# HanielUlises/GCN-GrabCut

Measured on AMD Instinct MI355X. Metric: images/sec end-to-end mask (DUTS-shape batch), higher is better.
Workload: dtype f32

## Files before the change

### gcn-grabcut_amd/csrc/ggc_gc.h

```cpp
#pragma once
#include "ggc_internal.h"

namespace ggc {

constexpr int DINF = 1 << 29;

struct GcDims { int B, H, W, P, n_chunks; };

__device__ __forceinline__ int dir_dx(int dir) { return (dir == 0 || dir == 4 || dir == 7) ? -1 : ((dir == 1 || dir == 5 || dir == 6) ? 1 : 0); }
__device__ __forceinline__ int dir_dy(int dir) { return (dir == 2 || dir == 4 || dir == 6) ? -1 : ((dir == 3 || dir == 5 || dir == 7) ? 1 : 0); }
__device__ __forceinline__ int dir_nb(const GcDims& d, int y, int x, int dir) {
    const int yy = y + dir_dy(dir), xx = x + dir_dx(dir);
    if (xx < 0 || xx >= d.W || yy < 0 || yy >= d.H) return -1;
    return yy * d.W + xx;
}

__host__ __device__ __forceinline__ size_t rc_idx(int dir, size_t i) { return i * 8 + (size_t)dir; }

__device__ __forceinline__ void mf_cold_pixel(size_t i, int32_t tw, const int32_t (&cap)[8], int32_t* __restrict__ rc,
                                              int32_t* __restrict__ ex, int32_t* __restrict__ snk, uint8_t* __restrict__ rmask) {
    int arcs = 0;
    int4* r = reinterpret_cast<int4*>(rc + rc_idx(0, i));
    r[0] = make_int4(cap[0], cap[1], cap[2], cap[3]);
    r[1] = make_int4(cap[4], cap[5], cap[6], cap[7]);
// ... 6 lines not shown

__device__ __forceinline__ void mf_plane_caps(const GcDims& d, int b, int p, const int32_t* __restrict__ nw, int32_t (&cap)[8]) {
    const size_t BP = (size_t)d.B * d.P;
    const int y = p / d.W, x = p % d.W;
    const int32_t* nwb = nw + (size_t)b * d.P;
    const int dirs[4] = {0, 4, 2, 6};
#pragma unroll
    for (int k = 0; k < 4; ++k) {
        const int dir = dirs[k];
        cap[dir] = dir_nb(d, y, x, dir) >= 0 ? nwb[(size_t)k * BP + p] : 0;
        const int q = dir_nb(d, y, x, dir ^ 1);
        cap[dir ^ 1] = q >= 0 ? nwb[(size_t)k * BP + q] : 0;
    }
}

__device__ __forceinline__ void mf_warm_pixel(size_t i, int32_t tw, int32_t tw_old, int32_t* __restrict__ ex,
                                              int32_t* __restrict__ snk) {
    const int32_t bal = (ex[i] - snk[i]) + (tw - tw_old);
    ex[i] = bal > 0 ? bal : 0;
    snk[i] = bal < 0 ? -bal : 0;
}

struct MfControl {
    int32_t* active;
    int32_t* cnt;
    int32_t* lists;
    int32_t* err;
};

int maxflow(ggc_ctx* ctx, hipStream_t st, const GcDims& d, const int32_t* state, int32_t* rc, int32_t* ex,
            int32_t* snk, int32_t* dist, uint8_t* rmask, const MfControl& ctl, bool masks_exact, int& n_open);

constexpr int MF_RT = 32;
constexpr int MF_PT_W = 32, MF_PT_H = 8;
struct MfTiles { int rt_x, rt_y, pt_x, pt_y; };
// ... 13 lines not shown
```

### gcn-grabcut_amd/csrc/ggc_grabcut.hip

```cpp
#include "ggc_gc.h"
#include "ggc_math.h"
#include <algorithm>
#include <cmath>
#include <cstdlib>
#include <vector>

namespace ggc {

constexpr int NCOMP = 5;
constexpr double CAP_SCALE = 262144.0;
constexpr double GAMMA = 50.0, LAMBDA = 9.0 * GAMMA;
constexpr int CHUNK = 1024;


struct Gmm {
    double coef[NCOMP], mean[NCOMP][3], cov[NCOMP][9];
    double inv[NCOMP][3][3], det[NCOMP];
    double isd[NCOMP];
};

__host__ __device__ inline void gmm_prepare(Gmm& g, int ci, double fix) {
    if (!(g.coef[ci] > 0.0)) return;
    double* c = g.cov[ci];
    double d = c[0] * (c[4] * c[8] - c[5] * c[7]) - c[1] * (c[3] * c[8] - c[5] * c[6]) + c[2] * (c[3] * c[7] - c[4] * c[6]);
// ... 3 lines not shown
    }
    g.det[ci] = d;
    g.isd[ci] = 1.0 / sqrt(d);
    const double id = 1.0 / d;
    g.inv[ci][0][0] = (c[4] * c[8] - c[5] * c[7]) * id;
    g.inv[ci][1][0] = -(c[3] * c[8] - c[5] * c[6]) * id;
    g.inv[ci][2][0] = (c[3] * c[7] - c[4] * c[6]) * id;
    g.inv[ci][0][1] = -(c[1] * c[8] - c[2] * c[7]) * id;
    g.inv[ci][1][1] = (c[0] * c[8] - c[2] * c[6]) * id;
    g.inv[ci][2][1] = -(c[0] * c[7] - c[1] * c[6]) * id;
    g.inv[ci][0][2] = (c[1] * c[5] - c[2] * c[4]) * id;
    g.inv[ci][1][2] = -(c[0] * c[5] - c[2] * c[3]) * id;
    g.inv[ci][2][2] = (c[0] * c[4] - c[1] * c[3]) * id;
}

__device__ __forceinline__ double gmm_comp(const Gmm& g, int ci, const uint8_t* px) {
    if (!(g.coef[ci] > 0.0)) return 0.0;
    const double d0 = (double)px[0] - g.mean[ci][0], d1 = (double)px[1] - g.mean[ci][1], d2 = (double)px[2] - g.mean[ci][2];
    const double mult = d0 * (d0 * g.inv[ci][0][0] + d1 * g.inv[ci][1][0] + d2 * g.inv[ci][2][0])
                      + d1 * (d0 * g.inv[ci][0][1] + d1 * g.inv[ci][1][1] + d2 * g.inv[ci][2][1])
                      + d2 * (d0 * g.inv[ci][0][2] + d1 * g.inv[ci][1][2] + d2 * g.inv[ci][2][2]);
    return g.isd[ci] * det_exp(-0.5 * mult);
}
__device__ __forceinline__ double gmm_total(const Gmm& g, const uint8_t* px) {
    double r = 0.0;
    for (int ci = 0; ci < NCOMP; ++ci) r += g.coef[ci] * gmm_comp(g, ci, px);
    return r;
}
__device__ __forceinline__ int gmm_which(const Gmm& g, const uint8_t* px) {
    int k = 0; double mx = 0.0;
    for (int ci = 0; ci < NCOMP; ++ci) { const double p = gmm_comp(g, ci, px); if (p > mx) { k = ci; mx = p; } }
    return k;
}

__device__ __forceinline__ bool is_bg(uint8_t m) { return m == GGC_BGD || m == GGC_PR_BGD; }

__global__ void __launch_bounds__(256) k_gc_flags(GcDims d, const uint8_t* __restrict__ mask, int32_t* __restrict__ flags) {
    const int b = blockIdx.y;
    int f = 0;
    for (int p = blockIdx.x * blockDim.x + threadIdx.x; p < d.P; p += gridDim.x * blockDim.x) {
        const uint8_t m = mask[(size_t)b * d.P + p];
        f |= (m == GGC_FGD) ? 1 : 0;
        f |= (m == GGC_BGD) ? 2 : 0;
        f |= (m > 3) ? 4 : 0;
        f |= is_bg(m) ? 8 : 16;
    }
    for (int o = 32; o > 0; o >>= 1) f |= __shfl_xor(f, o, 64);
    __shared__ int s_f[4];
    if ((threadIdx.x & 63) == 0) s_f[threadIdx.x >> 6] = f;
    __syncthreads();
    if (threadIdx.x == 0) {
        f = s_f[0] | s_f[1] | s_f[2] | s_f[3];
        if (f & ~__hip_atomic_load(&flags[b], __ATOMIC_RELAXED, __HIP_MEMORY_SCOPE_AGENT)) atomicOr(&flags[b], f);
    }
}

__global__ void __launch_bounds__(256) k_gc_promote(GcDims d, const int32_t* __restrict__ flags, uint8_t* __restrict__ mask) {
    const size_t i = (size_t)blockIdx.x * blockDim.x + threadIdx.x;
    if (i >= (size_t)d.B * d.P) return;
    const int f = flags[i / d.P];
    uint8_t m = mask[i];
    if (!(f & 1) && m == GGC_PR_FGD) m = GGC_FGD;
    if (!(f & 2) && m == GGC_PR_BGD) m = GGC_BGD;
    mask[i] = m;
}

__global__ void __launch_bounds__(256) k_gc_rect(GcDims d, const int32_t* __restrict__ rects, uint8_t* __restrict__ mask) {
    const size_t i = (size_t)blockIdx.x * blockDim.x + threadIdx.x;
    if (i >= (size_t)d.B * d.P) return;
    const int b = (int)(i / d.P), p = (int)(i % d.P);
    const int y = p / d.W, x = p % d.W;
    int x0 = rects[4 * b], y0 = rects[4 * b + 1], w = rects[4 * b + 2], h = rects[4 * b + 3];
    if (x0 < 0) { w += x0; x0 = 0; }
    if (y0 < 0) { h += y0; y0 = 0; }
    if (x0 + w > d.W) w = d.W - x0;
    if (y0 + h > d.H) h = d.H - y0;
    mask[i] = (x >= x0 && x < x0 + w && y >= y0 && y < y0 + h) ? GGC_PR_FGD : GGC_BGD;
}

__global__ void k_gc_state(int B, int mode, const int32_t* __restrict__ f1, const int32_t* __restrict__ f2,
                           int32_t* __restrict__ state, int32_t* __restrict__ err) {
    const int b = blockIdx.x * blockDim.x + threadIdx.x;
    if (b >= B) return;
    int s = 0;
    if ((f1[b] | f2[b]) & 4) { *err = 1; s = 1; }
    if (mode == 0 && (f2[b] & 3) != 3) s = 1;
    if (mode != 2 && (f2[b] & 24) != 24) s = 1;
    state[b] = s;
}

__device__ __forceinline__ uint64_t splitmix(uint64_t& s) {
    uint64_t z = (s += 0x9E3779B97F4A7C15ULL);
    z = (z ^ (z >> 30)) * 0xBF58476D1CE4E5B9ULL;
    z = (z ^ (z >> 27)) * 0x94D049BB133111EBULL;
    return z ^ (z >> 31);
}

struct KmState {
    uint64_t rng;
    int64_t n;
    int32_t K;
    int32_t cen_px[NCOMP];
    double cen[NCOMP][3];
};

__global__ void __launch_bounds__(256) k_km_chunks(GcDims d, int k, const uint8_t* __restrict__ img,
                                                   const uint8_t* __restrict__ mask, const int32_t* __restrict__ state,
                                                   const KmState* __restrict__ km, int32_t* __restrict__ d2,
                                                   int64_t* __restrict__ chunk_cnt, int64_t* __restrict__ chunk_d2) {
    __shared__ long long s_cnt[2][4], s_d2[2][4];
    const int b = blockIdx.y, ch = blockIdx.x, tid = threadIdx.x;
    if (state[b]) return;
    const uint8_t* im = img + (size_t)b * d.P * 3;
    long long cnt[2] = {0, 0}, sd[2] = {0, 0};
    for (int t = 0; t < CHUNK / 256; ++t) {
        const int p = ch * CHUNK + t * 256 + tid;
        if (p >= d.P) continue;
        const int c = is_bg(mask[(size_t)b * d.P + p]) ? 0 : 1;
        int v = 0;
        if (k > 0) {
            const KmState& s = km[b * 2 + c];
            if (k - 1 < s.K) {
                const int q = s.cen_px[k - 1];
                int dd = 0;
                for (int ch3 = 0; ch3 < 3; ++ch3) { const int t3 = (int)im[3 * p + ch3] - (int)im[3 * q + ch3]; dd += t3 * t3; }
                v = (k == 1) ? dd : min(d2[(size_t)b * d.P + p], dd);
                d2[(size_t)b * d.P + p] = v;
            } else v = d2[(size_t)b * d.P + p];
        }
        cnt[c] += 1; sd[c] += v;
    }
    for (int c = 0; c < 2; ++c)
        for (int o = 32; o > 0; o >>= 1) { cnt[c] += __shfl_xor(cnt[c], o, 64); sd[c] += __shfl_xor(sd[c], o, 64); }
    if ((tid & 63) == 0) for (int c = 0; c < 2; ++c) { s_cnt[c][tid >> 6] = cnt[c]; s_d2[c][tid >> 6] = sd[c]; }
    __syncthreads();
    if (tid < 2) {
        const size_t o = ((size_t)b * 2 + tid) * d.n_chunks + ch;
        chunk_cnt[o] = s_cnt[tid][0] + s_cnt[tid][1] + s_cnt[tid][2] + s_cnt[tid][3];
        chunk_d2[o] = s_d2[tid][0] + s_d2[tid][1] + s_d2[tid][2] + s_d2[tid][3];
    }
}

__device__ __forceinline__ long long wave_sum64(long long v) {
    for (int o = 32; o > 0; o >>= 1) v += __shfl_xor(v, o, 64);
    return v;
// ... 74 lines not shown
        s.rng = rng;
        s.cen_px[k] = pick;
        for (int ch3 = 0; ch3 < 3; ++ch3) s.cen[k][ch3] = (double)img[((size_t)b * d.P + pick) * 3 + ch3];
    }
}

constexpr int ACC_W = 13;

constexpr int BIN_COPIES = 16, BIN_PX = 4;

__global__ void __launch_bounds__(256) k_km_assign(GcDims d, const uint8_t* __restrict__ img,
                                                   const uint8_t* __restrict__ mask, const int32_t* __restrict__ state,
                                                   const KmState* __restrict__ km, uint8_t* __restrict__ comp,
                                                   unsigned long long* __restrict__ acc, int store_comp) {
    __shared__ unsigned int s_acc[2 * NCOMP * 4 * BIN_COPIES];
    const int b = blockIdx.y, tid = threadIdx.x, cp = tid % BIN_COPIES;
    if (state[b]) return;
    for (int i = tid; i < 2 * NCOMP * 4 * BIN_COPIES; i += 256) s_acc[i] = 0;
    __syncthreads();
#pragma unroll
    for (int j = 0; j < BIN_PX; ++j) {
        const int p = (blockIdx.x * BIN_PX + j) * 256 + tid;
        if (p < d.P) {
            const size_t gp = (size_t)b * d.P + p;
            const int c = is_bg(mask[gp]) ? 0 : 1;
            const uint8_t* px = img + gp * 3;
            int best = 0; double bd = 0.0;
#pragma unroll
            for (int cc = 0; cc < 2; ++cc) {
                if (c != cc) continue;
                const KmState& s = km[b * 2 + cc];
                for (int k = 0; k < s.K; ++k) {
                    const double a0 = (double)px[0] - s.cen[k][0], a1 = (double)px[1] - s.cen[k][1], a2 = (double)px[2] - s.cen[k][2];
                    const double dist = (a0 * a0 + a1 * a1) + a2 * a2;
                    if (k == 0 || dist < bd) { best = k; bd = dist; }
                }
            }
            if (store_comp) comp[gp] = (uint8_t)best;
            unsigned int* a = s_acc + (c * NCOMP + best) * 4 * BIN_COPIES + cp;
            atomicAdd(&a[0], 1u); atomicAdd(&a[BIN_COPIES], (unsigned int)px[0]);
            atomicAdd(&a[2 * BIN_COPIES], (unsigned int)px[1]); atomicAdd(&a[3 * BIN_COPIES], (unsigned int)px[2]);
        }
    }
    __syncthreads();
    for (int i = tid; i < 2 * NCOMP * 4; i += 256) {
        unsigned int v = 0;
#pragma unroll
        for (int k = 0; k < BIN_COPIES; ++k) v += s_acc[i * BIN_COPIES + k];
        if (v) atomicAdd(&acc[((size_t)b * 2 * NCOMP + i / 4) * ACC_W + (i % 4)], (unsigned long long)v);
    }
}

__global__ void k_km_update(int B, const int32_t* __restrict__ state, KmState* __restrict__ km,
                            unsigned long long* __restrict__ acc, int update) {
    const int i = blockIdx.x * blockDim.x + threadIdx.x;
    if (i >= B * 2 * NCOMP) return;
    const int b = i / (2 * NCOMP), c = (i / NCOMP) % 2, k = i % NCOMP;
    unsigned long long* a = acc + (size_t)i * ACC_W;
    if (!state[b] && update && a[0] > 0)
        for (int ch = 0; ch < 3; ++ch) km[b * 2 + c].cen[k][ch] = (double)(long long)a[1 + ch] / (double)(long long)a[0];
    for (int j = 0; j < ACC_W; ++j) a[j] = 0;
}

template <int MODE>
__global__ void __launch_bounds__(256) k_gmm_accum(GcDims d, const uint8_t* __restrict__ img,
                                                   uint8_t* __restrict__ mask, const int32_t* __restrict__ state,
                                                   const Gmm* __restrict__ gmm, const uint8_t* __restrict__ comp,
                                                   const int32_t* __restrict__ dist, unsigned long long* __restrict__ acc) {
    constexpr int LW = 10;
    __shared__ unsigned int s_acc[2 * NCOMP * LW * BIN_COPIES];
    const int b = blockIdx.y, tid = threadIdx.x, cp = tid % BIN_COPIES;
    if (state[b]) return;
    for (int i = tid; i < 2 * NCOMP * LW * BIN_COPIES; i += 256) s_acc[i] = 0;
    __syncthreads();
#pragma unroll
    for (int j = 0; j < BIN_PX; ++j) {
        const int p = (blockIdx.x * BIN_PX + j) * 256 + tid;
        if (p < d.P) {
            const size_t gp = (size_t)b * d.P + p;
            uint8_t m = mask[gp];
            if (MODE == 1 && dist && (m == GGC_PR_BGD || m == GGC_PR_FGD)) {
                const uint8_t m1 = dist[gp] >= DINF ? GGC_PR_FGD : GGC_PR_BGD;
                if (m1 != m) mask[gp] = m = m1;
            }
            const int c = is_bg(m) ? 0 : 1;
            const uint8_t* px = img + gp * 3;
            int ci = 0;
            if (MODE == 1) {
#pragma unroll
                for (int cc = 0; cc < 2; ++cc) if (c == cc) ci = gmm_which(gmm[b * 2 + cc], px);
            } else ci = comp[gp];
            unsigned int* a = s_acc + (c * NCOMP + ci) * LW * BIN_COPIES + cp;
            const unsigned int v0 = px[0], v1 = px[1], v2 = px[2];
            atomicAdd(&a[0], 1u);
            atomicAdd(&a[1 * BIN_COPIES], v0); atomicAdd(&a[2 * BIN_COPIES], v1); atomicAdd(&a[3 * BIN_COPIES], v2);
            atomicAdd(&a[4 * BIN_COPIES], v0 * v0); atomicAdd(&a[5 * BIN_COPIES], v0 * v1); atomicAdd(&a[6 * BIN_COPIES], v0 * v2);
            atomicAdd(&a[7 * BIN_COPIES], v1 * v1); atomicAdd(&a[8 * BIN_COPIES], v1 * v2); atomicAdd(&a[9 * BIN_COPIES], v2 * v2);
        }
    }
    __syncthreads();
    for (int i = tid; i < 2 * NCOMP * ACC_W; i += 256) {
        const int bin = i / ACC_W, slot = i % ACC_W;
        int ls = slot;
        if (slot >= 4) {
            const int r = (slot - 4) / 3, cc = (slot - 4) % 3;
            const int lo = r < cc ? r : cc, hi = r < cc ? cc : r;
            ls = 4 + (lo == 0 ? hi : (lo == 1 ? 2 + hi : 5));
        }
        unsigned int v = 0;
#pragma unroll
        for (int k = 0; k < BIN_COPIES; ++k) v += s_acc[(bin * LW + ls) * BIN_COPIES + k];
        if (v) atomicAdd(&acc[(size_t)b * 2 * NCOMP * ACC_W + i], (unsigned long long)v);
    }
}

__global__ void k_gmm_learn(int B, const int32_t* __restrict__ state, unsigned long long* __restrict__ acc,
                            Gmm* __restrict__ gmm) {
    const int i = blockIdx.x * blockDim.x + threadIdx.x;
    if (i >= B * 2) return;
    unsigned long long* a = acc + (size_t)i * NCOMP * ACC_W;
    if (!state[i / 2]) {
        Gmm& g = gmm[i];
        long long total = 0;
        for (int ci = 0; ci < NCOMP; ++ci) total += (long long)a[ci * ACC_W];
        for (int ci = 0; ci < NCOMP; ++ci) {
            const long long n = (long long)a[ci * ACC_W];
            if (n == 0) { g.coef[ci] = 0.0; continue; }
            const double inv_n = 1.0 / (double)n;
            g.coef[ci] = (double)n / (double)total;
            for (int r = 0; r < 3; ++r) g.mean[ci][r] = (double)(long long)a[ci * ACC_W + 1 + r] * inv_n;
            for (int r = 0; r < 3; ++r)
                for (int c = 0; c < 3; ++c)
                    g.cov[ci][3 * r + c] = (double)(long long)a[ci * ACC_W + 4 + 3 * r + c] * inv_n - g.mean[ci][r] * g.mean[ci][c];
            gmm_prepare(g, ci, 0.01);
        }
    }
    for (int j = 0; j < NCOMP * ACC_W; ++j) a[j] = 0;
}

__global__ void k_gmm_from_model(int B, const double* __restrict__ bgd, const double* __restrict__ fgd, Gmm* __restrict__ gmm) {
    const int i = blockIdx.x * blockDim.x + threadIdx.x;
    if (i >= B * 2) return;
// ... 4 lines not shown
    for (int k = 0; k < 45; ++k) g.cov[k / 9][k % 9] = m[4 * NCOMP + k];
    for (int ci = 0; ci < NCOMP; ++ci) gmm_prepare(g, ci, 0.0);
}

__global__ void k_gmm_to_model(int B, const int32_t* __restrict__ state, const Gmm* __restrict__ gmm,
                               double* __restrict__ bgd, double* __restrict__ fgd) {
    const int i = blockIdx.x * blockDim.x + threadIdx.x;
    if (i >= B * 2 || state[i / 2]) return;
    double* m = (i & 1 ? fgd : bgd) + (size_t)(i / 2) * 65;
    const Gmm& g = gmm[i];
    for (int k = 0; k < NCOMP; ++k) m[k] = g.coef[k];
    for (int k = 0; k < 15; ++k) m[NCOMP + k] = g.mean[k / 3][k % 3];
    for (int k = 0; k < 45; ++k) m[4 * NCOMP + k] = g.cov[k / 9][k % 9];
}

__device__ __forceinline__ bool plane_nb(const GcDims& d, int y, int x, int k, int& q) {
    const int dy = (k == 0) ? 0 : -1, dx = (k == 0 || k == 1) ? -1 : (k == 2 ? 0 : 1);
    const int yy = y + dy, xx = x + dx;
    if (xx < 0 || xx >= d.W || yy < 0) return false;
    q = yy * d.W + xx;
    return true;
}
__device__ __forceinline__ int colour_d2(const uint8_t* a, const uint8_t* b) {
    const int t0 = (int)a[0] - (int)b[0], t1 = (int)a[1] - (int)b[1], t2 = (int)a[2] - (int)b[2];
    return t0 * t0 + t1 * t1 + t2 * t2;
}

__global__ void __launch_bounds__(256) k_beta(GcDims d, const uint8_t* __restrict__ img, unsigned long long* __restrict__ bsum) {
    const int b = blockIdx.y;
    const uint8_t* im = img + (size_t)b * d.P * 3;
    unsigned long long s = 0;
    for (int p = blockIdx.x * blockDim.x + threadIdx.x; p < d.P; p += gridDim.x * blockDim.x) {
        const int y = p / d.W, x = p % d.W;
        for (int k = 0; k < 4; ++k) { int q; if (plane_nb(d, y, x, k, q)) s += (unsigned long long)colour_d2(im + 3 * p, im + 3 * q); }
    }
    for (int o = 32; o > 0; o >>= 1) s += __shfl_xor(s, o, 64);
    if ((threadIdx.x & 63) == 0 && s) atomicAdd(&bsum[b], s);
}

__device__ __forceinline__ double gc_beta(const GcDims& d, unsigned long long bsum) {
    const long long bs = (long long)bsum;
    return bs > 0 ? 1.0 / (2.0 * (double)bs / (double)(4ll * d.W * d.H - 3ll * d.W - 3ll * d.H + 2)) : 0.0;
}
__device__ __forceinline__ int32_t nlink_cap(double beta, bool diagonal, const uint8_t* a, const uint8_t* b) {
    const double gdiv = GAMMA / sqrt(2.0);
    const double wt = (diagonal ? gdiv : GAMMA) * det_exp(-beta * (double)colour_d2(a, b));
    return (int32_t)rint(wt * CAP_SCALE);
}

__global__ void __launch_bounds__(256) k_build_graph(GcDims d, const uint8_t* __restrict__ img,
                                                     const uint8_t* __restrict__ mask, const int32_t* __restrict__ state,
                                                     const Gmm* __restrict__ gmm, const unsigned long long* __restrict__ bsum,
                                                     int32_t* __restrict__ rc, int32_t* __restrict__ ex,
                                                     int32_t* __restrict__ snk, uint8_t* __restrict__ rmask,
                                                     int32_t* __restrict__ tws, int warm) {
    const int b = blockIdx.y, p = blockIdx.x * blockDim.x + threadIdx.x;
    if (p >= d.P || state[b]) return;
    const size_t i = (size_t)b * d.P + p;
    const uint8_t m = mask[i];
    if (warm && (m == GGC_BGD || m == GGC_FGD)) return;
    double dv;
    if (m == GGC_BGD) dv = -LAMBDA;
    else if (m == GGC_FGD) dv = LAMBDA;
    else {
        const uint8_t* px = img + i * 3;
        const double from_src = -det_log(gmm_total(gmm[b * 2 + 0], px));
        const double to_snk = -det_log(gmm_total(gmm[b * 2 + 1], px));
        dv = from_src - to_snk;
        if (dv != dv) dv = 0.0;
        if (dv > LAMBDA) dv = LAMBDA;
        if (dv < -LAMBDA) dv = -LAMBDA;
    }
    const int32_t tw = (int32_t)rint(dv * CAP_SCALE);
    if (warm) mf_warm_pixel(i, tw, tws[i], ex, snk);
    else {
        const uint8_t* im = img + (size_t)b * d.P * 3;
        const double beta = gc_beta(d, bsum[b]);
        const int y = p / d.W, x = p % d.W;
        int32_t cap[8];
#pragma unroll
        for (int dir = 0; dir < 8; ++dir) {
            const int q = dir_nb(d, y, x, dir);
            cap[dir] = q >= 0 ? nlink_cap(beta, dir >= 4, im + 3 * p, im + 3 * q) : 0;
        }
        mf_cold_pixel(i, tw, cap, rc, ex, snk, rmask);
    }
    tws[i] = tw;
}

// ... 17 lines not shown
extern "C" int ggc_grabcut(ggc_ctx* ctx, ggc_stream stream, int B, int H, int W, const uint8_t* image,
                           uint8_t* mask, const int32_t* rects, double* bgd_model, double* fgd_model,
                           int n_iter, int mode, uint64_t seed, uint8_t* binary) {
    if (!ctx) return GGC_E_INVALID_ARG;
    GGC_REQUIRE(ctx, B >= 1 && H >= 1 && W >= 1 && B <= 65535, GGC_E_SHAPE, "bad shape B=%d H=%d W=%d", B, H, W);
    GGC_REQUIRE(ctx, (size_t)H * W < (1u << 28), GGC_E_SHAPE, "image too large");
    GGC_REQUIRE(ctx, image && mask, GGC_E_INVALID_ARG, "null pointer");
    GGC_REQUIRE(ctx, mode >= 0 && mode <= 2, GGC_E_INVALID_ARG, "mode must be 0 (mask), 1 (rect) or 2 (eval)");
    GGC_REQUIRE(ctx, mode != 1 || rects, GGC_E_INVALID_ARG, "mode 1 needs rects");
    GGC_REQUIRE(ctx, mode != 2 || (bgd_model && fgd_model), GGC_E_INVALID_ARG, "mode 2 needs both models");
    GGC_HIP(ctx, hipSetDevice(ctx->device));
    hipStream_t st = reinterpret_cast<hipStream_t>(stream);
    GcDims d{B, H, W, H * W, cdiv((size_t)H * W, CHUNK)};
    const size_t BP = (size_t)B * d.P;

    int32_t *f1, *f2, *state, *err;
    MfControl mf;
    const size_t ctl_bytes = carve_scratch(ctx, S_GC_A, [&](Carve& c) {
        f1 = c.take<int32_t>(B); f2 = c.take<int32_t>(B); state = c.take<int32_t>(B); err = c.take<int32_t>(2);
        mf = {c.take<int32_t>(B), c.take<int32_t>(8), c.take<int32_t>(2 * (size_t)B), err ? err + 1 : nullptr};
    });
    Gmm* gmm = scratch_t<Gmm>(ctx, S_GC_B, (size_t)B * 2);
    unsigned long long* acc = scratch_t<unsigned long long>(ctx, S_GC_C, (size_t)B * 2 * NCOMP * ACC_W + B);
    uint8_t* comp = scratch_t<uint8_t>(ctx, S_GC_D, BP);
    int32_t* tws = scratch_t<int32_t>(ctx, S_GC_E, BP);
    int32_t* rc = scratch_t<int32_t>(ctx, S_GC_F, BP * 8);
    int32_t* ex = scratch_t<int32_t>(ctx, S_GC_G, BP * 3);
    uint8_t* rmask = scratch_t<uint8_t>(ctx, S_GC_L, BP);
    if (!ctl_bytes || !gmm || !acc || !comp || !tws || !rc || !ex || !rmask) return GGC_E_OOM;
    int32_t* snk = ex + BP;
    int32_t* dist = ex + 2 * BP;
    unsigned long long* bsum = acc + (size_t)B * 2 * NCOMP * ACC_W;
    GGC_HIP(ctx, hipMemsetAsync(f1, 0, ctl_bytes, st));
    GGC_HIP(ctx, hipMemsetAsync(acc, 0, sizeof(unsigned long long) * ((size_t)B * 2 * NCOMP * ACC_W + B), st));

    if (mode == 1) {
        int32_t* drects = scratch_t<int32_t>(ctx, S_GC_H, (size_t)B * 4);
        if (!drects) return GGC_E_OOM;
        GGC_HIP(ctx, hipMemcpyAsync(drects, rects, sizeof(int32_t) * B * 4, hipMemcpyHostToDevice, st));
        hipLaunchKernelGGL(k_gc_rect, dim3(cdiv(BP, 256)), dim3(256), 0, st, d, drects, mask);
    }
    const dim3 red(std::min(cdiv(d.P, 256 * 4), 128), B);
    hipLaunchKernelGGL(k_gc_flags, red, dim3(256), 0, st, d, mask, f1);
    if (mode == 0) hipLaunchKernelGGL(k_gc_promote, dim3(cdiv(BP, 256)), dim3(256), 0, st, d, f1, mask);
    hipLaunchKernelGGL(k_gc_flags, red, dim3(256), 0, st, d, mask, f2);
    hipLaunchKernelGGL(k_gc_state, dim3(cdiv(B, 256)), dim3(256), 0, st, B, mode, f1, f2, state, err);
    GGC_LAUNCH_CHECK(ctx);

    if (mode == 2) {
        hipLaunchKernelGGL(k_gmm_from_model, dim3(cdiv(B * 2, 64)), dim3(64), 0, st, B, bgd_model, fgd_model, gmm);
    } else {
        ProfScope prof(ctx, st, "grabcut_init_gmm");
        KmState* km = scratch_t<KmState>(ctx, S_GC_I, (size_t)B * 2);
        int32_t* d2 = scratch_t<int32_t>(ctx, S_GC_J, BP);
        int64_t* chunks = scratch_t<int64_t>(ctx, S_GC_K, (size_t)B * 2 * d.n_chunks * 2);
        if (!km || !d2 || !chunks) return GGC_E_OOM;
        int64_t* chunk_cnt = chunks;
        int64_t* chunk_d2 = chunks + (size_t)B * 2 * d.n_chunks;
        for (int k = 0; k < NCOMP; ++k) {
            hipLaunchKernelGGL(k_km_chunks, dim3(d.n_chunks, B), dim3(256), 0, st, d, k, image, mask, state, km, d2, chunk_cnt, chunk_d2);
            hipLaunchKernelGGL(k_km_pick, dim3(B), dim3(128), 0, st, d, k, (uint64_t)seed, image, mask, state, d2, chunk_cnt, chunk_d2, km);
        }
        for (int it = 0; it < 10; ++it) {
            hipLaunchKernelGGL(k_km_assign, dim3(cdiv(d.P, 256 * BIN_PX), B), dim3(256), 0, st, d, image, mask, state, km, comp, acc, it == 9 ? 1 : 0);
            hipLaunchKernelGGL(k_km_update, dim3(cdiv(B * 2 * NCOMP, 256)), dim3(256), 0, st, B, state, km, acc, it < 9 ? 1 : 0);
        }
        hipLaunchKernelGGL((k_gmm_accum<0>), dim3(cdiv(d.P, 256 * BIN_PX), B), dim3(256), 0, st, d, image, mask, state, gmm, comp, (const int32_t*)nullptr, acc);
        hipLaunchKernelGGL(k_gmm_learn, dim3(cdiv(B * 2, 64)), dim3(64), 0, st, B, state, acc, gmm);
    }
    GGC_LAUNCH_CHECK(ctx);

    if (n_iter > 0) {
        hipLaunchKernelGGL(k_beta, red, dim3(256), 0, st, d, image, bsum);
        GGC_LAUNCH_CHECK(ctx);
        int n_open = -1;
        for (int it = 0; it < n_iter; ++it) {
            const bool warm = knobs().mf_warm && it > 0;
            {
                ProfScope prof(ctx, st, "grabcut_gmm");
                hipLaunchKernelGGL((k_gmm_accum<1>), dim3(cdiv(d.P, 256 * BIN_PX), B), dim3(256), 0, st, d, image, mask, state, gmm, comp,
                                   (const int32_t*)(it > 0 ? dist : nullptr), acc);
                hipLaunchKernelGGL(k_gmm_learn, dim3(cdiv(B * 2, 64)), dim3(64), 0, st, B, state, acc, gmm);
                hipLaunchKernelGGL(k_build_graph, dim3(cdiv(d.P, 256), B), dim3(256), 0, st, d, image, mask, state, gmm, bsum, rc, ex, snk, rmask, tws, warm ? 1 : 0);
            }
            GGC_LAUNCH_CHECK(ctx);
            const int rcode = maxflow(ctx, st, d, state, rc, ex, snk, dist, rmask, mf, !warm, n_open);
            if (rcode) return rcode;
            if (it == n_iter - 1) hipLaunchKernelGGL(k_gc_relabel, dim3(cdiv(BP, 256)), dim3(256), 0, st, d, state, dist, mask);
            GGC_LAUNCH_CHECK(ctx);
        }
    }
    if (bgd_model && fgd_model)
        hipLaunchKernelGGL(k_gmm_to_model, dim3(cdiv(B * 2, 64)), dim3(64), 0, st, B, state, gmm, bgd_model, fgd_model);
    if (binary) hipLaunchKernelGGL(k_gc_binary, dim3(cdiv(BP, 256)), dim3(256), 0, st, BP, mask, binary);
    GGC_LAUNCH_CHECK(ctx);
    std::vector<int32_t> herr;
    int rcode = read_i32(ctx, st, err, 2, herr);
    if (rcode) return rcode;
// ... 5 lines not shown
```

Baseline: 3969.

## Vectorize GrabCut pixel kernels with 4-pixel quads and cache GMM assignments

```diff
diff --git a/gcn-grabcut_amd/csrc/ggc_gc.h b/gcn-grabcut_amd/csrc/ggc_gc.h
--- a/gcn-grabcut_amd/csrc/ggc_gc.h
+++ b/gcn-grabcut_amd/csrc/ggc_gc.h
@@ -44,11 +44,15 @@
     }
 }
 
+__device__ __forceinline__ void mf_warm_pixel(size_t i, int32_t tw, int32_t tw_old, int32_t ex_old, int32_t snk_old,
+                                              int32_t* __restrict__ ex, int32_t* __restrict__ snk) {
+    const int32_t bal = (ex_old - snk_old) + (tw - tw_old);
+    ex[i] = bal > 0 ? bal : 0;
+    snk[i] = bal < 0 ? -bal : 0;
+}
 __device__ __forceinline__ void mf_warm_pixel(size_t i, int32_t tw, int32_t tw_old, int32_t* __restrict__ ex,
                                               int32_t* __restrict__ snk) {
-    const int32_t bal = (ex[i] - snk[i]) + (tw - tw_old);
-    ex[i] = bal > 0 ? bal : 0;
-    snk[i] = bal < 0 ? -bal : 0;
+    mf_warm_pixel(i, tw, tw_old, ex[i], snk[i], ex, snk);
 }
 
 struct MfControl {
diff --git a/gcn-grabcut_amd/csrc/ggc_grabcut.hip b/gcn-grabcut_amd/csrc/ggc_grabcut.hip
--- a/gcn-grabcut_amd/csrc/ggc_grabcut.hip
+++ b/gcn-grabcut_amd/csrc/ggc_grabcut.hip
@@ -2,6 +2,7 @@
 #include "ggc_math.h"
 #include <algorithm>
 #include <cmath>
+#include <cstddef>
 #include <cstdlib>
 #include <vector>
 
@@ -41,37 +42,104 @@
     g.inv[ci][2][2] = (c[0] * c[4] - c[1] * c[3]) * id;
 }
 
-__device__ __forceinline__ double gmm_comp(const Gmm& g, int ci, const uint8_t* px) {
+struct GmmEval {
+    double coef[NCOMP], mean[NCOMP][3], inv[NCOMP][3][3], isd[NCOMP];
+};
+constexpr int GMM_EVAL_W = sizeof(GmmEval) / sizeof(double);
+static_assert(sizeof(Gmm) == 120 * sizeof(double) && GMM_EVAL_W == 70, "gmm_stage copies by double index");
+static_assert(offsetof(Gmm, coef) == 0 && offsetof(Gmm, mean) == 5 * sizeof(double) && offsetof(Gmm, inv) == 65 * sizeof(double) &&
+              offsetof(Gmm, isd) == 115 * sizeof(double), "gmm_stage's source offsets: coef, mean | inv | isd");
+static_assert(offsetof(GmmEval, inv) == 20 * sizeof(double) && offsetof(GmmEval, isd) == 65 * sizeof(double), "and its destinations");
+
+__device__ __forceinline__ void gmm_stage(GmmEval (&s)[2], const Gmm* __restrict__ g, int tid) {
+    if (tid < 2 * GMM_EVAL_W) {
+        const int c = tid / GMM_EVAL_W, k = tid % GMM_EVAL_W;
+        const int src = k < 20 ? k : (k < 65 ? k + 45 : k + 50);
+        reinterpret_cast<double*>(&s[c])[k] = reinterpret_cast<const double*>(&g[c])[src];
+    }
+}
+
+__device__ __forceinline__ double gmm_comp(const GmmEval& g, int ci, double c0, double c1, double c2) {
     if (!(g.coef[ci] > 0.0)) return 0.0;
-    const double d0 = (double)px[0] - g.mean[ci][0], d1 = (double)px[1] - g.mean[ci][1], d2 = (double)px[2] - g.mean[ci][2];
+    const double d0 = c0 - g.mean[ci][0], d1 = c1 - g.mean[ci][1], d2 = c2 - g.mean[ci][2];
     const double mult = d0 * (d0 * g.inv[ci][0][0] + d1 * g.inv[ci][1][0] + d2 * g.inv[ci][2][0])
                       + d1 * (d0 * g.inv[ci][0][1] + d1 * g.inv[ci][1][1] + d2 * g.inv[ci][2][1])
                       + d2 * (d0 * g.inv[ci][0][2] + d1 * g.inv[ci][1][2] + d2 * g.inv[ci][2][2]);
     return g.isd[ci] * det_exp(-0.5 * mult);
 }
-__device__ __forceinline__ double gmm_total(const Gmm& g, const uint8_t* px) {
-    double r = 0.0;
-    for (int ci = 0; ci < NCOMP; ++ci) r += g.coef[ci] * gmm_comp(g, ci, px);
+__device__ __forceinline__ double gmm_total(const GmmEval& g, double c0, double c1, double c2, int& which) {
+    double r = 0.0, mx = 0.0;
+    which = 0;
+    for (int ci = 0; ci < NCOMP; ++ci) {
+        const double p = gmm_comp(g, ci, c0, c1, c2);
+        r += g.coef[ci] * p;
+        if (p > mx) { which = ci; mx = p; }
+    }
     return r;
 }
-__device__ __forceinline__ int gmm_which(const Gmm& g, const uint8_t* px) {
+__device__ __forceinline__ int gmm_which(const GmmEval& g, double c0, double c1, double c2) {
     int k = 0; double mx = 0.0;
-    for (int ci = 0; ci < NCOMP; ++ci) { const double p = gmm_comp(g, ci, px); if (p > mx) { k = ci; mx = p; } }
+    for (int ci = 0; ci < NCOMP; ++ci) { const double p = gmm_comp(g, ci, c0, c1, c2); if (p > mx) { k = ci; mx = p; } }
     return k;
 }
 
 __device__ __forceinline__ bool is_bg(uint8_t m) { return m == GGC_BGD || m == GGC_PR_BGD; }
+
+struct Quad {
+    size_t g0;
+    int p0;
+    unsigned ok;
+};
+__host__ __device__ inline int quads_per_image(int P) { return (P + 3 + 3) / 4; }
+__device__ __forceinline__ Quad quad_of(const GcDims& d, int b, int q) {
+    const size_t base = (size_t)b * d.P;
+    Quad r;
+    r.g0 = (base & ~(size_t)3) + 4 * (size_t)q;
+    r.p0 = (int)((long long)r.g0 - (long long)base);
+    r.ok = 0;
+#pragma unroll
+    for (int j = 0; j < 4; ++j) r.ok |= (r.p0 + j >= 0 && r.p0 + j < d.P) ? 1u << j : 0u;
+    return r;
+}
+__device__ __forceinline__ bool dword_aligned(const void* p) { return (reinterpret_cast<uintptr_t>(p) & 3) == 0; }
+
+template <int N>
+__device__ __forceinline__ void quad_load(const uint8_t* __restrict__ base, const Quad& q, uint32_t (&w)[N]) {
+    const uint8_t* a = base + q.g0 * N;
+    if (q.ok == 15u && dword_aligned(base)) {
+        const uint32_t* a4 = reinterpret_cast<const uint32_t*>(a);
+#pragma unroll
+        for (int k = 0; k < N; ++k) w[k] = a4[k];
+    } else {
+#pragma unroll
+        for (int k = 0; k < N; ++k) w[k] = 0;
+#pragma unroll
+        for (int k = 0; k < 4 * N; ++k)
+            if ((q.ok >> (k / N)) & 1u) w[k >> 2] |= (uint32_t)a[k] << ((k & 3) * 8);
+    }
+}
+template <int N>
+__device__ __forceinline__ unsigned quad_byte(const uint32_t (&w)[N], int k) { return (w[k >> 2] >> ((k & 3) * 8)) & 255u; }
+
+__device__ __forceinline__ void quad_store(uint8_t* __restrict__ base, const Quad& q, uint32_t w) {
+    uint8_t* a = base + q.g0;
+    if (q.ok == 15u && dword_aligned(base)) *reinterpret_cast<uint32_t*>(a) = w;
+    else {
+#pragma unroll
+        for (int j = 0; j < 4; ++j) if ((q.ok >> j) & 1u) a[j] = (uint8_t)(w >> (8 * j));
+    }
+}
+
+__device__ __forceinline__ int mask_flags(unsigned m) {
+    if (m > 3u) return 4;
+    return (m == GGC_FGD ? 1 : 0) | (m == GGC_BGD ? 2 : 0) | ((m == GGC_BGD || m == GGC_PR_BGD) ? 8 : 16);
+}
 
 __global__ void __launch_bounds__(256) k_gc_flags(GcDims d, const uint8_t* __restrict__ mask, int32_t* __restrict__ flags) {
     const int b = blockIdx.y;
     int f = 0;
-    for (int p = blockIdx.x * blockDim.x + threadIdx.x; p < d.P; p += gridDim.x * blockDim.x) {
-        const uint8_t m = mask[(size_t)b * d.P + p];
-        f |= (m == GGC_FGD) ? 1 : 0;
-        f |= (m == GGC_BGD) ? 2 : 0;
-        f |= (m > 3) ? 4 : 0;
-        f |= is_bg(m) ? 8 : 16;
-    }
+    for (int p = blockIdx.x * blockDim.x + threadIdx.x; p < d.P; p += gridDim.x * blockDim.x)
+        f |= mask_flags(mask[(size_t)b * d.P + p]);
     for (int o = 32; o > 0; o >>= 1) f |= __shfl_xor(f, o, 64);
     __shared__ int s_f[4];
     if ((threadIdx.x & 63) == 0) s_f[threadIdx.x >> 6] = f;
@@ -83,13 +151,31 @@
 }
 
 __global__ void __launch_bounds__(256) k_gc_promote(GcDims d, const int32_t* __restrict__ flags, uint8_t* __restrict__ mask) {
-    const size_t i = (size_t)blockIdx.x * blockDim.x + threadIdx.x;
-    if (i >= (size_t)d.B * d.P) return;
-    const int f = flags[i / d.P];
-    uint8_t m = mask[i];
-    if (!(f & 1) && m == GGC_PR_FGD) m = GGC_FGD;
-    if (!(f & 2) && m == GGC_PR_BGD) m = GGC_BGD;
-    mask[i] = m;
+    const size_t BP = (size_t)d.B * d.P, i0 = 4 * ((size_t)blockIdx.x * blockDim.x + threadIdx.x);
+    if (i0 >= BP) return;
+    Quad q{i0, 0, 0};
+#pragma unroll
+    for (int j = 0; j < 4; ++j) q.ok |= i0 + j < BP ? 1u << j : 0u;
+    int bj = (int)(i0 / d.P), f[4];
+    size_t next = (size_t)(bj + 1) * d.P;
+    int all = 3;
+#pragma unroll
+    for (int j = 0; j < 4; ++j) {
+        while (i0 + j >= next && bj + 1 < d.B) { ++bj; next += d.P; }
+        f[j] = flags[bj];
+        if ((q.ok >> j) & 1u) all &= f[j];
+    }
+    if (all == 3) return;
+    uint32_t w[1];
+    quad_load<1>(mask, q, w);
+    uint32_t out = w[0];
+#pragma unroll
+    for (int j = 0; j < 4; ++j) {
+        const unsigned m = quad_byte<1>(w, j);
+        if (!(f[j] & 1) && m == GGC_PR_FGD) out = (out & ~(255u << (8 * j))) | ((uint32_t)GGC_FGD << (8 * j));
+        if (!(f[j] & 2) && m == GGC_PR_BGD) out = (out & ~(255u << (8 * j))) | ((uint32_t)GGC_BGD << (8 * j));
+    }
+    if (out != w[0]) quad_store(mask, q, out);
 }
 
 __global__ void __launch_bounds__(256) k_gc_rect(GcDims d, const int32_t* __restrict__ rects, uint8_t* __restrict__ mask) {
@@ -105,14 +191,17 @@
     mask[i] = (x >= x0 && x < x0 + w && y >= y0 && y < y0 + h) ? GGC_PR_FGD : GGC_BGD;
 }
 
-__global__ void k_gc_state(int B, int mode, const int32_t* __restrict__ f1, const int32_t* __restrict__ f2,
-                           int32_t* __restrict__ state, int32_t* __restrict__ err) {
+__host__ __device__ inline int flags_after_promotion(int f1) { return f1 | ((f1 & 16) ? 1 : 0) | ((f1 & 8) ? 2 : 0); }
+
+__global__ void k_gc_state(int B, int mode, const int32_t* __restrict__ f1, int32_t* __restrict__ state,
+                           int32_t* __restrict__ err) {
     const int b = blockIdx.x * blockDim.x + threadIdx.x;
     if (b >= B) return;
+    const int f2 = mode == 0 ? flags_after_promotion(f1[b]) : f1[b];
     int s = 0;
-    if ((f1[b] | f2[b]) & 4) { *err = 1; s = 1; }
-    if (mode == 0 && (f2[b] & 3) != 3) s = 1;
-    if (mode != 2 && (f2[b] & 24) != 24) s = 1;
+    if (f2 & 4) { *err = 1; s = 1; }
+    if (mode == 0 && (f2 & 3) != 3) s = 1;
+    if (mode != 2 && (f2 & 24) != 24) s = 1;
     state[b] = s;
 }
 
@@ -135,27 +224,52 @@
                                                    const uint8_t* __restrict__ mask, const int32_t* __restrict__ state,
                                                    const KmState* __restrict__ km, int32_t* __restrict__ d2,
                                                    int64_t* __restrict__ chunk_cnt, int64_t* __restrict__ chunk_d2) {
-    __shared__ long long s_cnt[2][4], s_d2[2][4];
+    __shared__ int s_cnt[2][4], s_d2[2][4];
     const int b = blockIdx.y, ch = blockIdx.x, tid = threadIdx.x;
     if (state[b]) return;
     const uint8_t* im = img + (size_t)b * d.P * 3;
-    long long cnt[2] = {0, 0}, sd[2] = {0, 0};
-    for (int t = 0; t < CHUNK / 256; ++t) {
-        const int p = ch * CHUNK + t * 256 + tid;
-        if (p >= d.P) continue;
-        const int c = is_bg(mask[(size_t)b * d.P + p]) ? 0 : 1;
-        int v = 0;
-        if (k > 0) {
+    const int lo = ch * CHUNK, hi = min(lo + CHUNK, d.P);
+    const int first = (int)((((size_t)b * d.P + lo) >> 2) - (((size_t)b * d.P) >> 2));
+    const int n_quads = (int)((((size_t)b * d.P + hi - 1) >> 2) - (((size_t)b * d.P) >> 2)) - first + 1;
+    bool upd[2] = {false, false};
+    int cq[2][3] = {{0, 0, 0}, {0, 0, 0}};
+    if (k > 0) {
+#pragma unroll
+        for (int c = 0; c < 2; ++c) {
             const KmState& s = km[b * 2 + c];
-            if (k - 1 < s.K) {
-                const int q = s.cen_px[k - 1];
-                int dd = 0;
-                for (int ch3 = 0; ch3 < 3; ++ch3) { const int t3 = (int)im[3 * p + ch3] - (int)im[3 * q + ch3]; dd += t3 * t3; }
-                v = (k == 1) ? dd : min(d2[(size_t)b * d.P + p], dd);
-                d2[(size_t)b * d.P + p] = v;
-            } else v = d2[(size_t)b * d.P + p];
-        }
-        cnt[c] += 1; sd[c] += v;
+            upd[c] = k - 1 < s.K;
+            if (upd[c]) { const int q = s.cen_px[k - 1]; for (int ch3 = 0; ch3 < 3; ++ch3) cq[c][ch3] = im[3 * q + ch3]; }
+        }
+    }
+    int cnt[2] = {0, 0}, sd[2] = {0, 0};
+    for (int t = tid; t < n_quads; t += 256) {
+        Quad q = quad_of(d, b, first + t);
+#pragma unroll
+        for (int j = 0; j < 4; ++j) if (q.p0 + j < lo || q.p0 + j >= hi) q.ok &= ~(1u << j);
+        uint32_t mw[1], cw[3];
+        quad_load<1>(mask, q, mw);
+        if (k > 0) quad_load<3>(img, q, cw);
+        int old[4] = {0, 0, 0, 0};
+        if (k > 1) {
+#pragma unroll
+            for (int j = 0; j < 4; ++j) if ((q.ok >> j) & 1u) old[j] = d2[q.g0 + j];
+        }
+#pragma unroll
+        for (int j = 0; j < 4; ++j) {
+            if (!((q.ok >> j) & 1u)) continue;
+            const int c = is_bg((uint8_t)quad_byte<1>(mw, j)) ? 0 : 1;
+            int v = 0;
+            if (k > 0) {
+                if (upd[c]) {
+                    int dd = 0;
+#pragma unroll
+                    for (int ch3 = 0; ch3 < 3; ++ch3) { const int t3 = (int)quad_byte<3>(cw, 3 * j + ch3) - cq[c][ch3]; dd += t3 * t3; }
+                    v = (k == 1) ? dd : min(old[j], dd);
+                    if (k == 1 || v != old[j]) d2[q.g0 + j] = v;
+                } else v = (k > 1) ? old[j] : d2[q.g0 + j];
+            }
+            cnt[c] += 1; sd[c] += v;
+        }
     }
     for (int c = 0; c < 2; ++c)
         for (int o = 32; o > 0; o >>= 1) { cnt[c] += __shfl_xor(cnt[c], o, 64); sd[c] += __shfl_xor(sd[c], o, 64); }
@@ -260,34 +374,40 @@
                                                    const KmState* __restrict__ km, uint8_t* __restrict__ comp,
                                                    unsigned long long* __restrict__ acc, int store_comp) {
     __shared__ unsigned int s_acc[2 * NCOMP * 4 * BIN_COPIES];
+    __shared__ double s_cen[2][NCOMP][3];
+    __shared__ int s_K[2];
     const int b = blockIdx.y, tid = threadIdx.x, cp = tid % BIN_COPIES;
     if (state[b]) return;
+    const Quad q = quad_of(d, b, blockIdx.x * 256 + tid);
+    uint32_t mw[1], cw[3];
+    quad_load<1>(mask, q, mw);
+    quad_load<3>(img, q, cw);
     for (int i = tid; i < 2 * NCOMP * 4 * BIN_COPIES; i += 256) s_acc[i] = 0;
+    if (tid < 2 * NCOMP * 3) s_cen[tid / (NCOMP * 3)][(tid / 3) % NCOMP][tid % 3] = km[b * 2 + tid / (NCOMP * 3)].cen[(tid / 3) % NCOMP][tid % 3];
+    if (tid >= 64 && tid < 66) s_K[tid - 64] = km[b * 2 + tid - 64].K;
     __syncthreads();
+    uint32_t cw_out = 0;
 #pragma unroll
     for (int j = 0; j < BIN_PX; ++j) {
-        const int p = (blockIdx.x * BIN_PX + j) * 256 + tid;
-        if (p < d.P) {
-            const size_t gp = (size_t)b * d.P + p;
-            const int c = is_bg(mask[gp]) ? 0 : 1;
-            const uint8_t* px = img + gp * 3;
+        if ((q.ok >> j) & 1u) {
+            const int c = is_bg((uint8_t)quad_byte<1>(mw, j)) ? 0 : 1;
+            const unsigned int v0 = quad_byte<3>(cw, 3 * j), v1 = quad_byte<3>(cw, 3 * j + 1), v2 = quad_byte<3>(cw, 3 * j + 2);
+            const double x0 = (double)v0, x1 = (double)v1, x2 = (double)v2;
             int best = 0; double bd = 0.0;
-#pragma unroll
-            for (int cc = 0; cc < 2; ++cc) {
-                if (c != cc) continue;
-                const KmState& s = km[b * 2 + cc];
-                for (int k = 0; k < s.K; ++k) {
-                    const double a0 = (double)px[0] - s.cen[k][0], a1 = (double)px[1] - s.cen[k][1], a2 = (double)px[2] - s.cen[k][2];
-                    const double dist = (a0 * a0 + a1 * a1) + a2 * a2;
-                    if (k == 0 || dist < bd) { best = k; bd = dist; }
-                }
+            const int K = s_K[c];
+#pragma unroll
+            for (int k = 0; k < NCOMP; ++k) {
+                const double a0 = x0 - s_cen[c][k][0], a1 = x1 - s_cen[c][k][1], a2 = x2 - s_cen[c][k][2];
+                const double dist = (a0 * a0 + a1 * a1) + a2 * a2;
+                if (k < K && (k == 0 || dist < bd)) { best = k; bd = dist; }
             }
-            if (store_comp) comp[gp] = (uint8_t)best;
+            cw_out |= (uint32_t)best << (8 * j);
             unsigned int* a = s_acc + (c * NCOMP + best) * 4 * BIN_COPIES + cp;
-            atomicAdd(&a[0], 1u); atomicAdd(&a[BIN_COPIES], (unsigned int)px[0]);
-            atomicAdd(&a[2 * BIN_COPIES], (unsigned int)px[1]); atomicAdd(&a[3 * BIN_COPIES], (unsigned int)px[2]);
-        }
-    }
+            atomicAdd(&a[0], 1u); atomicAdd(&a[BIN_COPIES], v0);
+            atomicAdd(&a[2 * BIN_COPIES], v1); atomicAdd(&a[3 * BIN_COPIES], v2);
+        }
+    }
+    if (store_comp && q.ok) quad_store(comp, q, cw_out);
     __syncthreads();
     for (int i = tid; i < 2 * NCOMP * 4; i += 256) {
         unsigned int v = 0;
@@ -312,38 +432,53 @@
 __global__ void __launch_bounds__(256) k_gmm_accum(GcDims d, const uint8_t* __restrict__ img,
                                                    uint8_t* __restrict__ mask, const int32_t* __restrict__ state,
                                                    const Gmm* __restrict__ gmm, const uint8_t* __restrict__ comp,
-                                                   const int32_t* __restrict__ dist, unsigned long long* __restrict__ acc) {
+                                                   const int32_t* __restrict__ dist, unsigned long long* __restrict__ acc,
+                                                   int use_comp) {
     constexpr int LW = 10;
     __shared__ unsigned int s_acc[2 * NCOMP * LW * BIN_COPIES];
+    __shared__ GmmEval s_g[2];
     const int b = blockIdx.y, tid = threadIdx.x, cp = tid % BIN_COPIES;
     if (state[b]) return;
+    const Quad q = quad_of(d, b, blockIdx.x * 256 + tid);
+    uint32_t mw[1], cw[3], kw[1] = {0};
+    quad_load<1>(mask, q, mw);
+    quad_load<3>(img, q, cw);
+    if (MODE == 0 || use_comp) quad_load<1>(comp, q, kw);
     for (int i = tid; i < 2 * NCOMP * LW * BIN_COPIES; i += 256) s_acc[i] = 0;
+    if (MODE == 1) gmm_stage(s_g, gmm + b * 2, tid);
     __syncthreads();
+    int dw[4] = {0, 0, 0, 0};
+    if (MODE == 1 && dist) {
+#pragma unroll
+        for (int j = 0; j < BIN_PX; ++j) {
+            const unsigned m = quad_byte<1>(mw, j);
+            if (((q.ok >> j) & 1u) && (m == GGC_PR_BGD || m == GGC_PR_FGD)) dw[j] = dist[q.g0 + j];
+        }
+    }
+    uint32_t mw_out = mw[0];
 #pragma unroll
     for (int j = 0; j < BIN_PX; ++j) {
-        const int p = (blockIdx.x * BIN_PX + j) * 256 + tid;
-        if (p < d.P) {
-            const size_t gp = (size_t)b * d.P + p;
-            uint8_t m = mask[gp];
-            if (MODE == 1 && dist && (m == GGC_PR_BGD || m == GGC_PR_FGD)) {
-                const uint8_t m1 = dist[gp] >= DINF ? GGC_PR_FGD : GGC_PR_BGD;
-                if (m1 != m) mask[gp] = m = m1;
+        if ((q.ok >> j) & 1u) {
+            uint8_t m = (uint8_t)quad_byte<1>(mw, j);
+            const bool probable = m == GGC_PR_BGD || m == GGC_PR_FGD;
+            if (MODE == 1 && dist && probable) {
+                m = dw[j] >= DINF ? GGC_PR_FGD : GGC_PR_BGD;
+                mw_out = (mw_out & ~(255u << (8 * j))) | ((uint32_t)m << (8 * j));
             }
             const int c = is_bg(m) ? 0 : 1;
-            const uint8_t* px = img + gp * 3;
-            int ci = 0;
-            if (MODE == 1) {
-#pragma unroll
-                for (int cc = 0; cc < 2; ++cc) if (c == cc) ci = gmm_which(gmm[b * 2 + cc], px);
-            } else ci = comp[gp];
+            const unsigned int v0 = quad_byte<3>(cw, 3 * j), v1 = quad_byte<3>(cw, 3 * j + 1), v2 = quad_byte<3>(cw, 3 * j + 2);
+            int ci;
+            if (MODE == 0) ci = (int)quad_byte<1>(kw, j);
+            else if (use_comp && probable) ci = (int)(quad_byte<1>(kw, j) >> (4 * c)) & 15;
+            else ci = gmm_which(s_g[c], (double)v0, (double)v1, (double)v2);
             unsigned int* a = s_acc + (c * NCOMP + ci) * LW * BIN_COPIES + cp;
-            const unsigned int v0 = px[0], v1 = px[1], v2 = px[2];
             atomicAdd(&a[0], 1u);
             atomicAdd(&a[1 * BIN_COPIES], v0); atomicAdd(&a[2 * BIN_COPIES], v1); atomicAdd(&a[3 * BIN_COPIES], v2);
             atomicAdd(&a[4 * BIN_COPIES], v0 * v0); atomicAdd(&a[5 * BIN_COPIES], v0 * v1); atomicAdd(&a[6 * BIN_COPIES], v0 * v2);
             atomicAdd(&a[7 * BIN_COPIES], v1 * v1); atomicAdd(&a[8 * BIN_COPIES], v1 * v2); atomicAdd(&a[9 * BIN_COPIES], v2 * v2);
         }
     }
+    if (MODE == 1 && mw_out != mw[0]) quad_store(mask, q, mw_out);
     __syncthreads();
     for (int i = tid; i < 2 * NCOMP * ACC_W; i += 256) {
         const int bin = i / ACC_W, slot = i % ACC_W;
@@ -361,7 +496,7 @@
 }
 
 __global__ void k_gmm_learn(int B, const int32_t* __restrict__ state, unsigned long long* __restrict__ acc,
-                            Gmm* __restrict__ gmm) {
+                            Gmm* __restrict__ gmm, int fresh) {
     const int i = blockIdx.x * blockDim.x + threadIdx.x;
     if (i >= B * 2) return;
     unsigned long long* a = acc + (size_t)i * NCOMP * ACC_W;
@@ -371,7 +506,11 @@
         for (int ci = 0; ci < NCOMP; ++ci) total += (long long)a[ci * ACC_W];
         for (int ci = 0; ci < NCOMP; ++ci) {
             const long long n = (long long)a[ci * ACC_W];
-            if (n == 0) { g.coef[ci] = 0.0; continue; }
+            if (n == 0) {
+                g.coef[ci] = 0.0;
+                if (fresh) { for (int r = 0; r < 3; ++r) g.mean[ci][r] = 0.0; for (int r = 0; r < 9; ++r) g.cov[ci][r] = 0.0; }
+                continue;
+            }
             const double inv_n = 1.0 / (double)n;
             g.coef[ci] = (double)n / (double)total;
             for (int r = 0; r < 3; ++r) g.mean[ci][r] = (double)(long long)a[ci * ACC_W + 1 + r] * inv_n;
@@ -406,25 +545,51 @@
     for (int k = 0; k < 45; ++k) m[4 * NCOMP + k] = g.cov[k / 9][k % 9];
 }
 
-__device__ __forceinline__ bool plane_nb(const GcDims& d, int y, int x, int k, int& q) {
-    const int dy = (k == 0) ? 0 : -1, dx = (k == 0 || k == 1) ? -1 : (k == 2 ? 0 : 1);
-    const int yy = y + dy, xx = x + dx;
-    if (xx < 0 || xx >= d.W || yy < 0) return false;
-    q = yy * d.W + xx;
-    return true;
-}
 __device__ __forceinline__ int colour_d2(const uint8_t* a, const uint8_t* b) {
     const int t0 = (int)a[0] - (int)b[0], t1 = (int)a[1] - (int)b[1], t2 = (int)a[2] - (int)b[2];
     return t0 * t0 + t1 * t1 + t2 * t2;
 }
 
 __global__ void __launch_bounds__(256) k_beta(GcDims d, const uint8_t* __restrict__ img, unsigned long long* __restrict__ bsum) {
-    const int b = blockIdx.y;
+    const int b = blockIdx.y, nq = quads_per_image(d.P);
     const uint8_t* im = img + (size_t)b * d.P * 3;
     unsigned long long s = 0;
-    for (int p = blockIdx.x * blockDim.x + threadIdx.x; p < d.P; p += gridDim.x * blockDim.x) {
-        const int y = p / d.W, x = p % d.W;
-        for (int k = 0; k < 4; ++k) { int q; if (plane_nb(d, y, x, k, q)) s += (unsigned long long)colour_d2(im + 3 * p, im + 3 * q); }
+    for (int g = blockIdx.x * blockDim.x + threadIdx.x; g < nq; g += gridDim.x * blockDim.x) {
+        const Quad q = quad_of(d, b, g);
+        if (!q.ok) continue;
+        uint32_t cw[3];
+        quad_load<3>(img, q, cw);
+        int nb[7][3];
+#pragma unroll
+        for (int i = 0; i < 7; ++i) {
+            const int pi = i == 0 ? q.p0 - 1 : q.p0 - d.W - 2 + i;
+            const bool in = pi >= 0 && pi < d.P;
+#pragma unroll
+            for (int ch = 0; ch < 3; ++ch) nb[i][ch] = in ? (int)im[3 * (size_t)(in ? pi : 0) + ch] : 0;
+        }
+        const int pf = q.p0 < 0 ? 0 : q.p0;
+        int y = pf / d.W, x = pf - y * d.W;
+        unsigned int sq = 0;
+#pragma unroll
+        for (int j = 0; j < 4; ++j) {
+            if (!((q.ok >> j) & 1u) ) continue;
+            int own[3], left[3];
+#pragma unroll
+            for (int ch = 0; ch < 3; ++ch) {
+                own[ch] = (int)quad_byte<3>(cw, 3 * j + ch);
+                left[ch] = j == 0 ? nb[0][ch] : (int)quad_byte<3>(cw, 3 * (j > 0 ? j - 1 : 0) + ch);
+            }
+            const bool ok4[4] = {x > 0, y > 0 && x > 0, y > 0, y > 0 && x + 1 < d.W};
+#pragma unroll
+            for (int k = 0; k < 4; ++k) {
+                int dd = 0;
+#pragma unroll
+                for (int ch = 0; ch < 3; ++ch) { const int t = own[ch] - (k == 0 ? left[ch] : nb[j + k][ch]); dd += t * t; }
+                sq += ok4[k] ? (unsigned int)dd : 0u;
+            }
+            if (++x == d.W) { x = 0; ++y; }
+        }
+        s += sq;
     }
     for (int o = 32; o > 0; o >>= 1) s += __shfl_xor(s, o, 64);
     if ((threadIdx.x & 63) == 0 && s) atomicAdd(&bsum[b], s);
@@ -445,26 +610,35 @@
                                                      const Gmm* __restrict__ gmm, const unsigned long long* __restrict__ bsum,
                                                      int32_t* __restrict__ rc, int32_t* __restrict__ ex,
                                                      int32_t* __restrict__ snk, uint8_t* __restrict__ rmask,
-                                                     int32_t* __restrict__ tws, int warm) {
+                                                     int32_t* __restrict__ tws, uint8_t* __restrict__ comp, int warm) {
+    __shared__ GmmEval s_g[2];
     const int b = blockIdx.y, p = blockIdx.x * blockDim.x + threadIdx.x;
-    if (p >= d.P || state[b]) return;
-    const size_t i = (size_t)b * d.P + p;
+    if (state[b]) return;
+    const size_t i = (size_t)b * d.P + (p < d.P ? p : 0);
     const uint8_t m = mask[i];
+    gmm_stage(s_g, gmm + b * 2, threadIdx.x);
+    __syncthreads();
+    if (p >= d.P) return;
     if (warm && (m == GGC_BGD || m == GGC_FGD)) return;
+    const unsigned int v0 = img[i * 3], v1 = img[i * 3 + 1], v2 = img[i * 3 + 2];
+    int32_t tw_old = 0, ex_old = 0, snk_old = 0;
+    if (warm) { tw_old = tws[i]; ex_old = ex[i]; snk_old = snk[i]; }
     double dv;
     if (m == GGC_BGD) dv = -LAMBDA;
     else if (m == GGC_FGD) dv = LAMBDA;
     else {
-        const uint8_t* px = img + i * 3;
-        const double from_src = -det_log(gmm_total(gmm[b * 2 + 0], px));
-        const double to_snk = -det_log(gmm_total(gmm[b * 2 + 1], px));
+        int k0, k1;
+        const double c0 = (double)v0, c1 = (double)v1, c2 = (double)v2;
+        const double from_src = -det_log(gmm_total(s_g[0], c0, c1, c2, k0));
+        const double to_snk = -det_log(gmm_total(s_g[1], c0, c1, c2, k1));
+        comp[i] = (uint8_t)(k0 | (k1 << 4));
         dv = from_src - to_snk;
         if (dv != dv) dv = 0.0;
         if (dv > LAMBDA) dv = LAMBDA;
         if (dv < -LAMBDA) dv = -LAMBDA;
     }
     const int32_t tw = (int32_t)rint(dv * CAP_SCALE);
-    if (warm) mf_warm_pixel(i, tw, tws[i], ex, snk);
+    if (warm) mf_warm_pixel(i, tw, tw_old, ex_old, snk_old, ex, snk);
     else {
         const uint8_t* im = img + (size_t)b * d.P * 3;
         const double beta = gc_beta(d, bsum[b]);
@@ -512,10 +686,10 @@
     GcDims d{B, H, W, H * W, cdiv((size_t)H * W, CHUNK)};
     const size_t BP = (size_t)B * d.P;
 
-    int32_t *f1, *f2, *state, *err;
+    int32_t *f1, *state, *err;
     MfControl mf;
     const size_t ctl_bytes = carve_scratch(ctx, S_GC_A, [&](Carve& c) {
-        f1 = c.take<int32_t>(B); f2 = c.take<int32_t>(B); state = c.take<int32_t>(B); err = c.take<int32_t>(2);
+        f1 = c.take<int32_t>(B); state = c.take<int32_t>(B); err = c.take<int32_t>(2);
         mf = {c.take<int32_t>(B), c.take<int32_t>(8), c.take<int32_t>(2 * (size_t)B), err ? err + 1 : nullptr};
     });
     Gmm* gmm = scratch_t<Gmm>(ctx, S_GC_B, (size_t)B * 2);
@@ -538,11 +712,11 @@
         GGC_HIP(ctx, hipMemcpyAsync(drects, rects, sizeof(int32_t) * B * 4, hipMemcpyHostToDevice, st));
         hipLaunchKernelGGL(k_gc_rect, dim3(cdiv(BP, 256)), dim3(256), 0, st, d, drects, mask);
     }
-    const dim3 red(std::min(cdiv(d.P, 256 * 4), 128), B);
+    const int quad_blocks = cdiv(quads_per_image(d.P), 256);
+    const dim3 red(std::min(cdiv(d.P, 256 * 4), 128), B), dense(quad_blocks, B);
     hipLaunchKernelGGL(k_gc_flags, red, dim3(256), 0, st, d, mask, f1);
-    if (mode == 0) hipLaunchKernelGGL(k_gc_promote, dim3(cdiv(BP, 256)), dim3(256), 0, st, d, f1, mask);
-    hipLaunchKernelGGL(k_gc_flags, red, dim3(256), 0, st, d, mask, f2);
-    hipLaunchKernelGGL(k_gc_state, dim3(cdiv(B, 256)), dim3(256), 0, st, B, mode, f1, f2, state, err);
+    if (mode == 0) hipLaunchKernelGGL(k_gc_promote, dim3(cdiv(cdiv(BP, 4), 256)), dim3(256), 0, st, d, f1, mask);
+    hipLaunchKernelGGL(k_gc_state, dim3(cdiv(B, 256)), dim3(256), 0, st, B, mode, f1, state, err);
     GGC_LAUNCH_CHECK(ctx);
 
     if (mode == 2) {
@@ -560,11 +734,11 @@
             hipLaunchKernelGGL(k_km_pick, dim3(B), dim3(128), 0, st, d, k, (uint64_t)seed, image, mask, state, d2, chunk_cnt, chunk_d2, km);
         }
         for (int it = 0; it < 10; ++it) {
-            hipLaunchKernelGGL(k_km_assign, dim3(cdiv(d.P, 256 * BIN_PX), B), dim3(256), 0, st, d, image, mask, state, km, comp, acc, it == 9 ? 1 : 0);
+            hipLaunchKernelGGL(k_km_assign, dense, dim3(256), 0, st, d, image, mask, state, km, comp, acc, it == 9 ? 1 : 0);
             hipLaunchKernelGGL(k_km_update, dim3(cdiv(B * 2 * NCOMP, 256)), dim3(256), 0, st, B, state, km, acc, it < 9 ? 1 : 0);
         }
-        hipLaunchKernelGGL((k_gmm_accum<0>), dim3(cdiv(d.P, 256 * BIN_PX), B), dim3(256), 0, st, d, image, mask, state, gmm, comp, (const int32_t*)nullptr, acc);
-        hipLaunchKernelGGL(k_gmm_learn, dim3(cdiv(B * 2, 64)), dim3(64), 0, st, B, state, acc, gmm);
+        hipLaunchKernelGGL((k_gmm_accum<0>), dense, dim3(256), 0, st, d, image, mask, state, gmm, comp, (const int32_t*)nullptr, acc, 0);
+        hipLaunchKernelGGL(k_gmm_learn, dim3(cdiv(B * 2, 64)), dim3(64), 0, st, B, state, acc, gmm, 1);
     }
     GGC_LAUNCH_CHECK(ctx);
 
@@ -576,10 +750,10 @@
             const bool warm = knobs().mf_warm && it > 0;
             {
                 ProfScope prof(ctx, st, "grabcut_gmm");
-                hipLaunchKernelGGL((k_gmm_accum<1>), dim3(cdiv(d.P, 256 * BIN_PX), B), dim3(256), 0, st, d, image, mask, state, gmm, comp,
-                                   (const int32_t*)(it > 0 ? dist : nullptr), acc);
-                hipLaunchKernelGGL(k_gmm_learn, dim3(cdiv(B * 2, 64)), dim3(64), 0, st, B, state, acc, gmm);
-                hipLaunchKernelGGL(k_build_graph, dim3(cdiv(d.P, 256), B), dim3(256), 0, st, d, image, mask, state, gmm, bsum, rc, ex, snk, rmask, tws, warm ? 1 : 0);
+                hipLaunchKernelGGL((k_gmm_accum<1>), dense, dim3(256), 0, st, d, image, mask, state, gmm, comp,
+                                   (const int32_t*)(it > 0 ? dist : nullptr), acc, it > 0 ? 1 : 0);
+                hipLaunchKernelGGL(k_gmm_learn, dim3(cdiv(B * 2, 64)), dim3(64), 0, st, B, state, acc, gmm, 0);
+                hipLaunchKernelGGL(k_build_graph, dim3(cdiv(d.P, 256), B), dim3(256), 0, st, d, image, mask, state, gmm, bsum, rc, ex, snk, rmask, tws, comp, warm ? 1 : 0);
             }
             GGC_LAUNCH_CHECK(ctx);
             const int rcode = maxflow(ctx, st, d, state, rc, ex, snk, dist, rmask, mf, !warm, n_open);
```

Result: faster. 4048 (median of 6 runs) (+2.0%).
